# fhausmann/deepgrp

Hardware: AMD Instinct MI355X
Metric: Mbp/sec predicted (whole node) at window=200 stride=50, 5-class (higher is better)
Workload: dtype f16

## Files before the change

deepgrp_amd/csrc/api.hip:

```cpp
#include "dgrp_model.h"

#include <stdarg.h>
#include <string.h>

#include <algorithm>
#include <vector>
#include <mutex>

static thread_local char g_err[512] = "";

void dgrp_set_error(const char *fmt, ...)
{
    va_list ap;
    va_start(ap, fmt);
    vsnprintf(g_err, sizeof(g_err), fmt, ap);
    va_end(ap);
}

DGRP_EXPORT int dgrp_abi_version(void) { return DGRP_ABI_VERSION; }
DGRP_EXPORT const char *dgrp_last_error(void) { return g_err; }

DGRP_EXPORT int dgrp_device_info(char *name, size_t name_cap, int *cu_count, int64_t *hbm_bytes)
{
    int dev = 0;
// ... 553 lines not shown
    if (m->ref_only) {
        *kernel = DGRP_KERNEL_FP32; *lds_bytes = 0; *ospan = 0; *avg_up = 0;
        return DGRP_OK;
    }
    const dgrp_gru_plan plan = dgrp_gru_plan_for(m, mode, step);
    *kernel = (int)plan.kernel; *lds_bytes = (int64_t)plan.lds; *ospan = plan.ospan; *avg_up = plan.avg_up;
    return DGRP_OK;
}

DGRP_EXPORT int dgrp_model_set_precision(dgrp_model *m, int level)
{
    DGRP_REQUIRE(m, "dgrp_model_set_precision: NULL model");
    DGRP_REQUIRE(level == 0 || level == 1, "dgrp_model_set_precision: level must be 0 (fp16 operands) or 1 (split operands)");
    if (m->ref_only) return DGRP_OK;
    DGRP_REQUIRE(level == 0 || m->d_pack_lo || m->d_stream, "dgrp_model_set_precision: this model has no split-operand kernel");
    m->precision = level;
    return DGRP_OK;
}

static int64_t ref_sub_windows(const dgrp_model *m)
{
    const int64_t per = 2 * (int64_t)m->T * m->u * 4 + (int64_t)m->T * (m->C + 1) * 4 + 2 * (int64_t)m->u * 4;
    return std::max<int64_t>(16, std::min<int64_t>(4096, (512ll << 20) / per) / 16 * 16);
}

DGRP_EXPORT int64_t dgrp_forward_workspace_bytes(const dgrp_model *m, int64_t nw)
{
    if (!m || nw < 0) return 0;
    if (m->ref_only) {
        const int64_t sub = std::min<int64_t>(ref_sub_windows(m), std::max<int64_t>(nw, 1));
        return dgrp_align_up(dgrp_forward_reference_workspace_bytes(m, sub), 256) + dgrp_align_up(sub * m->T * (int64_t)m->C * 4, 256);
    }
    if (!m->attention) return 256;
    return dgrp_align_up(nw * m->T * (int64_t)m->UP * 4, 256) + dgrp_align_up(nw * m->T * (int64_t)m->C * 4, 256);
}

static int forward_ref(const dgrp_model *m, const uint8_t *d_idx, int64_t n, int64_t s, dgrp_placement place, int64_t w0, int64_t nw,
                       int merge, float *d_out, void *d_work, int64_t work_bytes, hipStream_t stream)
{
    if (work_bytes < dgrp_forward_workspace_bytes(m, nw) || !d_work) {
        dgrp_set_error("dgrp_forward: this model runs on the fp32 kernels and needs %lld bytes of workspace for %lld windows",
                       (long long)dgrp_forward_workspace_bytes(m, nw), (long long)nw);
        return DGRP_ENOMEM;
    }
    const int64_t sub = std::min<int64_t>(ref_sub_windows(m), nw);
    const int64_t ref_bytes = dgrp_align_up(dgrp_forward_reference_workspace_bytes(m, sub), 256);
    float *probs = (float *)((char *)d_work + ref_bytes);
    for (int64_t a = w0; a < w0 + nw; a += sub) {
        const int64_t k = std::min<int64_t>(sub, w0 + nw - a);
        float *dst = merge ? probs : d_out + (a - w0) * (int64_t)m->T * m->C;
        int rc = dgrp_forward_windows_reference(m, d_idx, n, s, a, k, dst, d_work, ref_bytes, stream);
        if (rc) return rc;
        if (!merge) continue;
        for (int64_t b = a; b < a + k;) {
            const int64_t e = (b < place.nfullB && a + k > place.nfullB) ? place.nfullB : a + k;
            const int64_t row = dgrp_place_row(place, b, s);
            if (row < n) {
                rc = dgrp_get_max(d_out + row * m->C, n - row, probs + (b - a) * (int64_t)m->T * m->C, m->T, m->C, s, e - b, stream);
                if (rc) return rc;
            }
            b = e;
        }
    }
    return DGRP_OK;
}

static int forward_common(const dgrp_model *m, const uint8_t *d_idx, int64_t n, int64_t s, int64_t batch, int64_t w0,
                          int64_t nw, int merge, float *d_out, void *d_work, int64_t work_bytes, hipStream_t stream)
{
    DGRP_REQUIRE(m && s >= 1 && w0 >= 0 && nw >= 0 && n >= 0, "dgrp_forward: bad arguments");
    if (nw == 0) return DGRP_OK;
    DGRP_REQUIRE(d_idx && d_out, "dgrp_forward: NULL pointer");
    DGRP_REQUIRE((w0 + nw - 1) * s + m->T <= n, "dgrp_forward: window %lld (start %lld) runs past n=%lld",
                 (long long)(w0 + nw - 1), (long long)((w0 + nw - 1) * s), (long long)n);
    dgrp_placement place = { 0, 0 };
    if (merge) {
        DGRP_REQUIRE(batch >= 1, "dgrp_forward_merge: batch must be >= 1");
        const int64_t total = dgrp_window_count(n, m->T, s);
        DGRP_REQUIRE(w0 + nw <= total, "dgrp_forward_merge: windows %lld..%lld exceed the record's %lld",
                     (long long)w0, (long long)(w0 + nw), (long long)total);
        place = dgrp_make_placement(total, batch);
    }
    if (m->ref_only) return forward_ref(m, d_idx, n, s, place, w0, nw, merge, d_out, d_work, work_bytes, stream);
    if (!m->attention) return dgrp_gru_launch(m, dgrp_gru_plan_for(m, merge ? 0 : 1, s), d_idx, n, place, w0, nw, d_out, nullptr, stream);
    if (work_bytes < dgrp_forward_workspace_bytes(m, nw) || !d_work) {
        dgrp_set_error("dgrp_forward: attention model needs %lld bytes of workspace for %lld windows",
                       (long long)dgrp_forward_workspace_bytes(m, nw), (long long)nw);
        return DGRP_ENOMEM;
    }
    void *avg = d_work;
    float *pl = (float *)((char *)d_work + dgrp_align_up(nw * m->T * (int64_t)m->UP * 4, 256));
    const dgrp_gru_plan pre = dgrp_gru_plan_for(m, 2, s);
    int rc = dgrp_gru_launch(m, pre, d_idx, n, place, w0, nw, pl, avg, stream);
    if (rc) return rc;
    return dgrp_attention_launch_recs(m, pre, place, w0, nw, merge, n, avg, pl, d_out, nullptr, 0, stream);
}

DGRP_EXPORT int dgrp_forward_windows(const dgrp_model *m, const uint8_t *d_idx, int64_t n, int64_t s, int64_t w0,
                                     int64_t nw, float *d_probs, void *d_work, int64_t work_bytes, void *stream)
{
    return forward_common(m, d_idx, n, s, 1, w0, nw, 0, d_probs, d_work, work_bytes, (hipStream_t)stream);
}

DGRP_EXPORT int dgrp_forward_merge(const dgrp_model *m, const uint8_t *d_idx, int64_t n, int64_t s, int64_t batch,
                                   int64_t w0, int64_t nw, float *d_out, void *d_work, int64_t work_bytes, void *stream)
{
    return forward_common(m, d_idx, n, s, batch, w0, nw, 1, d_out, d_work, work_bytes, (hipStream_t)stream);
}

static int64_t spill_cap_bytes()
{
    static const int64_t cap = [] {
        if (const char *e = getenv("DGRP_SPILL_BYTES")) {
            const long long v = atoll(e);
            if (v >= (1ll << 20)) return (int64_t)v;
        }
        size_t free_b = 0, total_b = 0;
        if (hipMemGetInfo(&free_b, &total_b) != hipSuccess || total_b == 0) return (int64_t)(4ll << 30);
        return std::min<int64_t>(8ll << 30, std::max<int64_t>(1ll << 30, (int64_t)(total_b / 32)));
    }();
    return cap;
}

static int64_t record_window_chunk(const dgrp_model *m)
{
    if (m->ref_only) return ref_sub_windows(m);
// ... 150 lines not shown
        dgrp_set_error("dgrp_predict_record: workspace %lld < %lld bytes", (long long)work_bytes, (long long)l.bytes);
        return DGRP_ENOMEM;
    }
    char *w = (char *)d_work;
    float *out = (float *)(w + l.out);
    int8_t *labels = (int8_t *)(w + l.labels);
    int64_t *d_count = (int64_t *)(w + l.count);
    DGRP_HIP(hipMemsetAsync(out, 0, (size_t)n * m->C * 4, stream));
    int rc = dgrp_forward_merge_record(m, d_idx, n, s, batch, out, w + l.fwd, l.fwd_bytes, stream);
    if (rc) return rc;
    if (use_mss) {
        rc = dgrp_scores(out, n, m->C, (double *)(w + l.scores), (int8_t *)(w + l.cls), stream);
        if (rc) return rc;
        rc = dgrp_mss_labels((const double *)(w + l.scores), (const int8_t *)(w + l.cls), n, m->C, min_mss_len, xdrop_len,
                             labels, nullptr, w + l.post, l.post_bytes, stream);
    } else {
        rc = dgrp_softmax_labels(out, n, m->C, nullptr, labels, w + l.post, l.post_bytes, stream);
    }
    if (rc) return rc;
    rc = dgrp_segments(labels, n, offset, contig, d_records, cap, d_count, w + l.post, l.post_bytes, stream);
    if (rc) return rc;
    DGRP_HIP(hipMemcpyAsync(h_count, d_count, 8, hipMemcpyDeviceToHost, stream));
    DGRP_HIP(hipStreamSynchronize(stream));
    return DGRP_OK;
}

int dgrp_batch_marks(const int64_t *d_start, const int64_t *d_len, int64_t nrec, int64_t total_n, uint8_t *d_marks,
                     double *d_scores, int8_t *d_cls, hipStream_t stream);
int dgrp_batch_segments(const int8_t *d_labels, const uint8_t *d_marks, int64_t total_n, const int64_t *d_start, int64_t nrec,
                        const int64_t *d_startpos, const int32_t *d_contig, dgrp_segment *d_records, int64_t cap,
                        int64_t *d_count, void *d_work, int64_t work_bytes, hipStream_t stream);

struct batch_layout {
    int64_t out, scores, cls, labels, marks, count, recs, wgf, start, len, spos, contig, post, post_bytes, avg, pl, bytes;
};

static batch_layout batch_carve(const dgrp_model *m, int64_t nrec, int64_t total_rows, int64_t total_windows)
{
    batch_layout l;
    int64_t p = 0;
    auto take = [&](int64_t b) { const int64_t q = p; p += dgrp_align_up(b, 256); return q; };
    l.out = take(total_rows * m->C * 4);
    l.scores = take(total_rows * 8);
    l.cls = take(total_rows);
    l.labels = take(total_rows);
    l.marks = take(total_rows);
    l.count = take(8);
    l.recs = take(nrec * 64);
    l.wgf = take((nrec + 1) * 8);
    l.start = take((nrec + 1) * 8);
    l.len = take(nrec * 8);
    l.spos = take(nrec * 8);
    l.contig = take(nrec * 4);
    l.post_bytes = std::max<int64_t>(std::max<int64_t>(dgrp_mss_batch_workspace_bytes(total_rows, nrec), dgrp_segments_workspace_bytes(total_rows)), 4096);
    l.post = take(l.post_bytes);
    l.avg = take(m->attention ? total_windows * m->T * (int64_t)m->UP * 4 : 0);
    l.pl = take(m->attention ? total_windows * m->T * (int64_t)m->C * 4 : 0);
    l.bytes = p;
    return l;
}

static int64_t batch_windows(const dgrp_model *m, int64_t nrec, const int64_t *h_n, int64_t s)
{
    int64_t w = 0;
    for (int64_t r = 0; r < nrec; ++r) w += dgrp_window_count(h_n[r], m->T, s);
    return w;
}

static int64_t batch_rows(int64_t nrec, const int64_t *h_n)
{
    int64_t rows = 0;
    for (int64_t r = 0; r < nrec; ++r) rows += dgrp_align_up(h_n[r], 64);
    return rows;
}

DGRP_EXPORT int64_t dgrp_batch_workspace_bytes(const dgrp_model *m, int64_t nrec, const int64_t *h_n, int64_t s)
{
    if (!m || nrec < 0 || s < 1 || (nrec > 0 && !h_n)) return 0;
    for (int64_t r = 0; r < nrec; ++r)
        if (h_n[r] < 1) return 0;
    return batch_carve(m, nrec, batch_rows(nrec, h_n), batch_windows(m, nrec, h_n, s)).bytes;
}

DGRP_EXPORT int64_t dgrp_batch_rows(int64_t nrec, const int64_t *h_n)
{
    return nrec > 0 && h_n ? batch_rows(nrec, h_n) : 0;
}

static int predict_batch_common(const char *who, const dgrp_model *m, const uint8_t *d_idx, int64_t nrec, const int64_t *h_idx_off,
                                const int64_t *h_n, const int64_t *h_startpos, const int32_t *h_contig, int64_t s,
// ... 9 lines not shown
        DGRP_REQUIRE(h_n[r] >= 1 && h_idx_off[r] >= 0, "%s: record %lld: empty records do not belong in a batch", who, (long long)r);
    const int64_t rows = batch_rows(nrec, h_n);
    DGRP_REQUIRE(rows < (1ll << 31), "%s: %lld rows in one batch (limit 2^31)", who, (long long)rows);
    const int64_t windows = batch_windows(m, nrec, h_n, s);
    DGRP_REQUIRE(windows < (1ll << 31), "%s: too many windows in one batch", who);
    const batch_layout l = batch_carve(m, nrec, rows, windows);
    if (work_bytes < l.bytes) {
        dgrp_set_error("%s: workspace %lld < %lld bytes", who, (long long)work_bytes, (long long)l.bytes);
        return DGRP_ENOMEM;
    }
    char *w = (char *)d_work;
    std::vector<int64_t> recs((size_t)nrec * 8, 0), wgf((size_t)nrec + 1, 0), start((size_t)nrec + 1, 0);
    int64_t wfirst = 0;
    for (int64_t r = 0; r < nrec; ++r) {
        const int64_t nwin = dgrp_window_count(h_n[r], m->T, s);
        const dgrp_placement pl = dgrp_make_placement(nwin, batch);
        int64_t *e = recs.data() + (size_t)r * 8;
        e[0] = h_idx_off[r]; e[1] = h_n[r]; e[2] = start[(size_t)r]; e[3] = nwin; e[4] = pl.nfullB; e[5] = pl.shift; e[6] = wfirst;
        wfirst += nwin;
        wgf[(size_t)r + 1] = wgf[(size_t)r] + (nwin + 15) / 16;
        start[(size_t)r + 1] = start[(size_t)r] + dgrp_align_up(h_n[r], 64);
    }
    DGRP_HIP(hipMemcpyAsync(w + l.recs, recs.data(), recs.size() * 8, hipMemcpyHostToDevice, stream));
    DGRP_HIP(hipMemcpyAsync(w + l.wgf, wgf.data(), wgf.size() * 8, hipMemcpyHostToDevice, stream));
    DGRP_HIP(hipMemcpyAsync(w + l.start, start.data(), start.size() * 8, hipMemcpyHostToDevice, stream));
    DGRP_HIP(hipMemcpyAsync(w + l.len, h_n, (size_t)nrec * 8, hipMemcpyHostToDevice, stream));
    DGRP_HIP(hipMemcpyAsync(w + l.spos, h_startpos, (size_t)nrec * 8, hipMemcpyHostToDevice, stream));
    DGRP_HIP(hipMemcpyAsync(w + l.contig, h_contig, (size_t)nrec * 4, hipMemcpyHostToDevice, stream));
    float *out = d_probs ? d_probs : (float *)(w + l.out);
    DGRP_HIP(hipMemsetAsync(out, 0, (size_t)rows * m->C * 4, stream));
    int rc;
    if (!m->attention) {
        rc = dgrp_gru_launch_batch(m, dgrp_gru_plan_for(m, 0, s), d_idx, w + l.recs, (const int64_t *)(w + l.wgf), nrec, wgf[(size_t)nrec],
                                   out, nullptr, stream);
        if (rc) return rc;
    } else {
        const dgrp_gru_plan pre = dgrp_gru_plan_for(m, 2, s);
        rc = dgrp_gru_launch_batch(m, pre, d_idx, w + l.recs, (const int64_t *)(w + l.wgf), nrec, wgf[(size_t)nrec], (float *)(w + l.pl),
                                   w + l.avg, stream);
        if (rc) return rc;
        rc = dgrp_attention_launch_recs(m, pre, dgrp_placement{ 0, 0 }, 0, windows, 1, rows, w + l.avg, (const float *)(w + l.pl), out,
                                        w + l.recs, nrec, stream);
        if (rc) return rc;
    }
    double *scores = (double *)(w + l.scores);
    int8_t *cls = (int8_t *)(w + l.cls), *labels = (int8_t *)(w + l.labels);
    uint8_t *marks = (uint8_t *)(w + l.marks);
    rc = dgrp_scores(out, rows, m->C, scores, cls, stream);
    if (rc) return rc;
    rc = dgrp_batch_marks((const int64_t *)(w + l.start), (const int64_t *)(w + l.len), nrec, rows, marks, scores, cls, stream);
    if (rc) return rc;
    rc = dgrp_mss_labels_batch(scores, cls, rows, nrec, start.data(), m->C, min_mss_len, xdrop_len, labels, w + l.post, l.post_bytes, stream);
    if (rc) return rc;
    int64_t *d_count = (int64_t *)(w + l.count);
    rc = dgrp_batch_segments(labels, marks, rows, (const int64_t *)(w + l.start), nrec, (const int64_t *)(w + l.spos),
                             (const int32_t *)(w + l.contig), d_records, cap, d_count, w + l.post, l.post_bytes, stream);
    if (rc) return rc;
    DGRP_HIP(hipMemcpyAsync(h_count, d_count, 8, hipMemcpyDeviceToHost, stream));
    DGRP_HIP(hipStreamSynchronize(stream));
    return DGRP_OK;
}

DGRP_EXPORT int dgrp_predict_batch(const dgrp_model *m, const uint8_t *d_idx, int64_t nrec, const int64_t *h_idx_off,
                                   const int64_t *h_n, const int64_t *h_startpos, const int32_t *h_contig, int64_t s,
                                   int64_t batch, int min_mss_len, int xdrop_len, dgrp_segment *d_records, int64_t cap,
                                   int64_t *h_count, void *d_work, int64_t work_bytes, void *stream)
{
    return predict_batch_common("dgrp_predict_batch", m, d_idx, nrec, h_idx_off, h_n, h_startpos, h_contig, s, batch, min_mss_len, xdrop_len,
                                d_records, cap, h_count, d_work, work_bytes, (hipStream_t)stream, nullptr);
}

DGRP_EXPORT int dgrp_predict_batch_probs(const dgrp_model *m, const uint8_t *d_idx, int64_t nrec, const int64_t *h_idx_off,
// ... 10 lines not shown
```

deepgrp_amd/csrc/dgrp_model.h:

```cpp
#pragma once
#include "dgrp_common.h"

struct dgrp_model {
    int T, u, C, attention;
    int cell;
    int onercp;
    int UP;
    int NW;
    int KS;
    int nfrag;
    int precision;
    int is_view;
    int ref_only;
    uint4 *d_pack;
    uint4 *d_pack_lo;
    uint4 *d_pack16;
    float *d_xtab;
    uint4 *d_stream;
    uint4 *d_packw;
    float *d_xtabw;
    int NU16;
    float *d_ffb;
    float *d_scale;
    float *d_wtop;
    float *d_raw;
    int64_t raw_kernel, raw_rec, raw_bias, raw_ffk, raw_ffb, raw_scale;
};

struct dgrp_timer_scope {
    hipStream_t stream;
    int64_t windows;
    hipEvent_t start;
    bool on;
    dgrp_timer_scope(hipStream_t s, int64_t nw);
    ~dgrp_timer_scope();
};

enum class dgrp_kernel { none, wave, split2, stream64, stream, split, lstm, fused };
struct dgrp_gru_plan {
    dgrp_kernel kernel;
    int mode;
    int64_t s;
    size_t lds;
    int ospan, lo_tile_off, xtab_off;
    int avg_up;
};
dgrp_gru_plan dgrp_gru_plan_for(const dgrp_model *m, int mode, int64_t s);
int dgrp_gru_launch(const dgrp_model *m, const dgrp_gru_plan &plan, const uint8_t *d_idx, int64_t n, dgrp_placement place,
                    int64_t w0, int64_t nw, float *d_out, void *d_avg, hipStream_t stream);
struct gru_params;
int dgrp_stream_launch(const gru_params &p, int cell, int NW, int64_t groups, size_t lds, hipStream_t stream);
int dgrp_wave_carve(int NU, gru_params &p, int mode, int64_t s, int64_t budget);
int dgrp_wave_table_bytes(int NU);
int dgrp_wave_launch(const gru_params &p, int NU, int64_t groups, int wave_bytes, bool onercp, hipStream_t stream);
size_t dgrp_stream64_carve(int NW, gru_params &p, int mode, int64_t s, int64_t budget);
int dgrp_stream64_launch(const gru_params &p, int NW, int64_t groups, size_t lds, hipStream_t stream);
int dgrp_gru_launch_batch(const dgrp_model *m, const dgrp_gru_plan &plan, const uint8_t *d_idx, const void *d_recs,
                          const int64_t *d_wg_first, int64_t nrec, int64_t total_groups, float *d_out, void *d_avg, hipStream_t stream);
int dgrp_attention_launch_recs(const dgrp_model *m, const dgrp_gru_plan &pre, dgrp_placement place, int64_t w0, int64_t nw,
                               int merge, int64_t n, const void *d_avg, const float *d_pl, float *d_out,
                               const void *d_recs, int64_t nrec, hipStream_t stream);
```

deepgrp_amd/csrc/gru_kernel.hip:

```cpp
#include "gru_shared.h"
#include <mutex>
template <int NW, int MODE, bool ONERCP>
__global__ void __launch_bounds__(64 * NW, 2) gru_fused_kernel(const gru_params pin)
{
    gru_params p = pin;
    const int64_t bid = wg_record<MODE>(pin, p);
    constexpr int UP = 32 * NW, KS = UP / 16, HS = UP + 8;
    constexpr bool ZSTREAM = NW > 4;
    extern __shared__ __attribute__((aligned(16))) unsigned char smem[];

    const int tid = threadIdx.x;
    const int lane = tid & 63;
    const int wave = __builtin_amdgcn_readfirstlane(tid >> 6);
    const int T = p.T, C = p.C;
    const uint4 *mypack = p.pack + (size_t)wave * p.nfrag * 64 + lane;
    half8 Bz[KS + 1], Br[KS + 1], Bg[KS + 1], Bxh, Bd_hi, Bd_lo;
#pragma unroll
    for (int k = 0; k <= KS; ++k) {
        uint4 a = mypack[(size_t)(k) * 64], b = mypack[(size_t)(KS + 1 + k) * 64], c = mypack[(size_t)(2 * (KS + 1) + k) * 64];
        if (!ZSTREAM || k == KS) Bz[k] = __builtin_bit_cast(half8, a);
        Br[k] = __builtin_bit_cast(half8, b);
        Bg[k] = __builtin_bit_cast(half8, c);
    }
    Bxh = __builtin_bit_cast(half8, mypack[(size_t)(3 * (KS + 1)) * 64]);
// ... 996 lines not shown
        set((const void *)lstm_fused_kernel<NW, 0>);
        set((const void *)lstm_fused_kernel<NW, 1>);
    });
    DGRP_HIP(cfg_err);
    if (p.mode == 0)
        hipLaunchKernelGGL((lstm_fused_kernel<NW, 0>), dim3((unsigned)groups), dim3(64 * NW), lds, stream, p);
    else
        hipLaunchKernelGGL((lstm_fused_kernel<NW, 1>), dim3((unsigned)groups), dim3(64 * NW), lds, stream, p);
    DGRP_LAUNCH_CHECK();
    return DGRP_OK;
}

static size_t gru_tile_carve(const dgrp_model *m, gru_params &p, int mode, int64_t s, bool split, int pad, int64_t budget)
{
    const int lo_tiles = split ? gru_lds_hbuf(m->UP, pad) : 0;
    const int fixed = gru_lds_hbuf(m->UP, pad) + gru_lds_dpart(m->NW) + gru_lds_seq(p.Tp) + gru_lds_meta();
    p.ospan = 0;
    if (mode == 0) {
        const int64_t want = (DGRP_WG_WINDOWS - 1) * s + m->T;
        const int64_t cap = (budget - fixed - lo_tiles) / (m->C * 4);
        p.ospan = (int)(want < cap ? want : cap);
        if (p.ospan < m->T) p.ospan = 0;
    }
    p.lo_tile_off = (int)dgrp_align_up(fixed + (int64_t)p.ospan * m->C * 4, 16);
    return split ? (size_t)p.lo_tile_off + lo_tiles : (size_t)fixed + (size_t)p.ospan * m->C * 4;
}
static int64_t tile_budget(const dgrp_model *m, bool split)
{
    if (m->NW == 1) return 19 * 1024;
    if (m->NW == 2 && split) return 39 * 1024;
    return (m->NW > 4 ? 144 : 72) * 1024;
}
#define DGRP_SPLIT2_PAD 16
#define DGRP_SPLIT2_XTAB_BYTES (5 * (4 * 128 * 4 + 32))

dgrp_gru_plan dgrp_gru_plan_for(const dgrp_model *m, int mode, int64_t s)
{
    gru_params p{};
    p.T = m->T; p.C = m->C; p.Tp = (int)dgrp_align_up(m->T, 16);
    dgrp_gru_plan plan{};
    plan.mode = mode; plan.s = s; plan.avg_up = m->UP;
    auto pick = [&](dgrp_kernel k, size_t lds) {
        plan.kernel = k; plan.lds = lds;
        plan.ospan = p.ospan; plan.lo_tile_off = p.lo_tile_off; plan.xtab_off = p.xtab_off;
        return plan;
    };
    const bool split = (m->cell == 1 && m->NW > 4 && m->d_stream) ||
                       (m->precision == 1 && ((m->cell == 0 && m->NW <= 4 && m->d_pack_lo) || m->d_stream));
    const bool one_tile = getenv("DGRP_SPLIT_ONE_TILE") != nullptr;
    if (split && !one_tile && m->cell == 0 && m->NU16 > 0 && m->d_packw && !(m->NU16 == 2 && mode == 2)) {
        const int64_t budget = (160 * 1024 - dgrp_wave_table_bytes(m->NU16)) / 4 / 16 * 16;
        const int wave_bytes = dgrp_wave_carve(m->NU16, p, mode, s, budget);
        if (wave_bytes <= budget) {
            plan.avg_up = 16 * m->NU16;
            return pick(dgrp_kernel::wave, wave_bytes);
        }
    }
    if (split && !one_tile && m->NW == 4 && m->d_pack16) {
        const int half_bytes = (int)dgrp_align_up((int64_t)gru_tile_carve(m, p, mode, s, true, DGRP_SPLIT2_PAD, 74 * 1024), 256);
        if (2 * half_bytes + DGRP_SPLIT2_XTAB_BYTES <= 160 * 1024) {
            p.xtab_off = 2 * half_bytes;
            return pick(dgrp_kernel::split2, half_bytes);
        }
    }
    const size_t lds = gru_tile_carve(m, p, mode, s, split, 8, tile_budget(m, split));
    if (lds > 160 * 1024) return pick(dgrp_kernel::none, lds);
    if (split && m->d_stream && m->cell == 0 && m->d_xtab) {
// ... 29 lines not shown
        case 3: return launch_split<3>(p, groups, plan.lds, stream);
        default: return launch_split<4>(p, groups, plan.lds, stream);
        }
    case dgrp_kernel::lstm:
        switch (m->NW) {
        case 1: return launch_lstm<1>(p, groups, plan.lds, stream);
        case 2: return launch_lstm<2>(p, groups, plan.lds, stream);
        case 3: return launch_lstm<3>(p, groups, plan.lds, stream);
        case 4: return launch_lstm<4>(p, groups, plan.lds, stream);
        default:
            dgrp_set_error("LSTM units=%d not supported (max 128)", m->u);
            return DGRP_EINVAL;
        }
    case dgrp_kernel::fused:
        switch (m->NW) {
        case 1: return launch_gru<1>(p, groups, plan.lds, onercp, stream);
        case 2: return launch_gru<2>(p, groups, plan.lds, onercp, stream);
        case 3: return launch_gru<3>(p, groups, plan.lds, onercp, stream);
        case 4: return launch_gru<4>(p, groups, plan.lds, onercp, stream);
        case 5: return launch_gru<5>(p, groups, plan.lds, onercp, stream);
        case 6: return launch_gru<6>(p, groups, plan.lds, onercp, stream);
        case 7: return launch_gru<7>(p, groups, plan.lds, onercp, stream);
        case 8: return launch_gru<8>(p, groups, plan.lds, onercp, stream);
        default:
            dgrp_set_error("units=%d not supported by the GRU kernel (max 256)", m->u);
            return DGRP_EINVAL;
        }
    }
    dgrp_set_error("window size %d: the workgroup's staged sequences (%d bytes of LDS) do not fit 160 KiB", m->T, gru_lds_seq(p.Tp));
    return DGRP_EINVAL;
}

int dgrp_gru_launch(const dgrp_model *m, const dgrp_gru_plan &plan, const uint8_t *d_idx, int64_t n, dgrp_placement place,
                    int64_t w0, int64_t nw, float *d_out, void *d_avg, hipStream_t stream)
{
    if (nw <= 0) return DGRP_OK;
    dgrp_timer_scope timed(stream, nw);
    gru_params p{};
    p.idx = d_idx; p.n = n; p.w0 = w0; p.nw = nw; p.place = place; p.out = d_out; p.avg = d_avg;
    const int64_t groups = (nw + DGRP_WG_WINDOWS - 1) / DGRP_WG_WINDOWS;
    DGRP_REQUIRE(groups < (1ll << 31), "too many windows in one launch (%lld)", (long long)nw);
    return gru_dispatch(m, plan, p, groups, stream);
}

int dgrp_gru_launch_batch(const dgrp_model *m, const dgrp_gru_plan &plan, const uint8_t *d_idx, const void *d_recs,
                          const int64_t *d_wg_first, int64_t nrec, int64_t total_groups, float *d_out, void *d_avg, hipStream_t stream)
{
    if (nrec <= 0 || total_groups <= 0) return DGRP_OK;
    dgrp_timer_scope timed(stream, total_groups * DGRP_WG_WINDOWS);
    DGRP_REQUIRE(m->NW <= 8 && (plan.mode == 0 || (plan.mode == 2 && m->cell == 0)), "dgrp_gru_launch_batch: mode 0, or the GRU attention pre-pass");
    gru_params p{};
    p.idx = d_idx; p.out = d_out; p.avg = d_avg;
    p.recs = (const gru_rec *)d_recs; p.wg_first = d_wg_first; p.nrec = nrec;
    DGRP_REQUIRE(total_groups < (1ll << 31), "too many windows in one launch");
    return gru_dispatch(m, plan, p, total_groups, stream);
}

int dgrp_attention_launch_recs(const dgrp_model *m, const dgrp_gru_plan &pre, dgrp_placement place, int64_t w0, int64_t nw,
                               int merge, int64_t n, const void *d_avg, const float *d_pl, float *d_out,
                               const void *d_recs, int64_t nrec, hipStream_t stream)
{
    if (nw <= 0) return DGRP_OK;
    const int64_t s = pre.s;
    att_params p;
    p.avg = d_avg; p.pl = d_pl; p.scale = m->d_scale; p.wtop = m->d_wtop; p.out = d_out;
    p.n = n; p.s = s; p.w0 = w0; p.nw = nw; p.place = place;
    p.T = m->T; p.C = m->C; p.UP = pre.avg_up; p.merge = merge;
    p.recs = (const gru_rec *)d_recs; p.nrec = nrec;
    const int UPs = p.UP;
    const bool f32 = m->precision == 1;
    const int esz = f32 ? 4 : 2;
    DGRP_REQUIRE(nw < (1ll << 31), "too many windows in one launch");
    p.ospan = 0;
    const int64_t want = (ATT_WPB - 1) * s + m->T;
    const unsigned grid = (unsigned)((nw + ATT_WPB - 1) / ATT_WPB);
    if (UPs <= 64) {
        const int stat = 4 * UPs * 2 * 4 + 4 * 64 * (UPs + 16 / esz) * esz;
        if (merge) {
            const int64_t budget = stat <= 40 * 1024 && !f32 ? 78 * 1024 : 156 * 1024;
            const int64_t cap = (budget - stat) / (m->C * 4);
            p.ospan = (int)(want < cap ? want : cap);
            if (p.ospan < m->T) p.ospan = 0;
        }
        const size_t dyn = (size_t)p.ospan * m->C * 4;
        static std::once_flag configured;
// ... 45 lines not shown
```

deepgrp_amd/csrc/gru_shared.h:

```cpp
#pragma once
#include "dgrp_model.h"

typedef _Float16 half8 __attribute__((ext_vector_type(8)));
typedef float f32x16 __attribute__((ext_vector_type(16)));
typedef float f32x4 __attribute__((ext_vector_type(4)));
typedef _Float16 half4 __attribute__((ext_vector_type(4)));

#define DGRP_WG_WINDOWS 16

struct gru_rec {
    int64_t idx_off, n, out_row, nwin;
    dgrp_placement place;
    int64_t win_first;
    int64_t pad_;
};

struct gru_params {
    const uint8_t *idx;
    int64_t n, s, w0, nw;
    dgrp_placement place;
    const uint4 *pack;
    const float *ffb;
    float *out;
    void *avg;
    int avg_f32;
    int T, C, nfrag, mode;
    int Tp;
    int ospan;
    const struct gru_rec *recs;
    const int64_t *wg_first;
    int64_t nrec;
    int64_t avgw;
    const uint4 *pack_lo;
    int lo_tile_off;
    float zfold;
    const uint4 *pack16;
    const float *xtab;
    int xtab_off;
    const uint4 *stream;
    const uint4 *packw;
    const float *xtabw;
    int avg_up;
};

__device__ __forceinline__ float sigmoid_from_scaled(float a) { return __builtin_amdgcn_rcpf(1.0f + __builtin_amdgcn_exp2f(a)); }
__device__ __forceinline__ float tanh_from_scaled(float a) { return 1.0f - 2.0f * __builtin_amdgcn_rcpf(1.0f + __builtin_amdgcn_exp2f(a)); }
typedef float f32x2 __attribute__((ext_vector_type(2)));
__device__ __forceinline__ f32x2 rcp1p_exp2_pair(float a0, float a1)
{
    f32x2 e = { __builtin_amdgcn_exp2f(a0), __builtin_amdgcn_exp2f(a1) };
    e = e + 1.0f;
    return f32x2{ __builtin_amdgcn_rcpf(e.x), __builtin_amdgcn_rcpf(e.y) };
}
__device__ __forceinline__ float fast_tanh(float x) { return tanh_from_scaled(2.8853900817779268f * x); }

template <int N>
__device__ __forceinline__ float row_ror(float x)
{
    return __builtin_bit_cast(float, __builtin_amdgcn_update_dpp(0, __builtin_bit_cast(int, x), 0x120 | N, 0xf, 0xf, false));
}
template <int N>
__device__ __forceinline__ float row_max_ror(float x)
{
    float r;
    asm("s_nop 1\n\tv_max_f32_dpp %0, %1, %1 row_ror:%2 row_mask:0xf bank_mask:0xf" : "=v"(r) : "v"(x), "n"(N));
    return r;
}
template <int CTRL>
__device__ __forceinline__ float quad_perm(float x)
{
    return __builtin_bit_cast(float, __builtin_amdgcn_update_dpp(0, __builtin_bit_cast(int, x), CTRL, 0xf, 0xf, false));
// ... 268 lines not shown
```

deepgrp_amd/csrc/gru_split2.hip:

```cpp
#include "gru_shared.h"
#include <cstddef>
#include <mutex>
#include <type_traits>

typedef unsigned u32x4 __attribute__((ext_vector_type(4)));

namespace {

constexpr int NW = 4, UP = 128, KS = 4, HPAD = 16, HS = UP + HPAD;
constexpr int XT_PITCH = 4 * 128 * 4 + 32;

struct split2_weights {
    u32x4 hi[3][KS][2], lo[3][KS][2];
    u32x4 Bd_hi, Bd_lo;
};

#define LOAD2(a, pa, b, pb)                                                                                             \
    asm volatile("global_load_dwordx4 %0, %2, off\n\tglobal_load_dwordx4 %1, %3, off"                                   \
                 : "=&a"(a), "=&a"(b) : "v"(pa), "v"(pb) : "memory")
#define LOAD_WAIT asm volatile("s_waitcnt vmcnt(0)" ::: "memory")

#define MFMA_R(acc, Wf, b) asm volatile("v_mfma_f32_16x16x32_f16 %0, %1, %2, %0" : "+v"(acc) : "a"(Wf), "v"(b))
#define MFMA_D(acc, a, Wf) asm volatile("v_mfma_f32_16x16x32_f16 %0, %1, %2, %0" : "+v"(acc) : "v"(a), "a"(Wf))
#define MFMA_DZ(acc, a, Wf) asm volatile("v_mfma_f32_16x16x32_f16 %0, %1, %2, 0" : "=&v"(acc) : "v"(a), "a"(Wf))

struct tile_state {
    gru_params p;
    wg_ctx ctx;
    unsigned hcur, hnxt, lcur, lnxt;
    unsigned myseq;
    float h[16];
    f32x4 ar[4], ag[4], az[4], ax[4];
    f32x4 dpl;
    unsigned tabf, tabr;
    half8 f0h[2], f0l[2];
    int p_off;
    int64_t p_row0;
    bool pr_on;
};

__device__ __forceinline__ int64_t split2_uniform(int64_t v)
{
    const unsigned lo = (unsigned)__builtin_amdgcn_readfirstlane((int)(uint64_t)v), hi = (unsigned)__builtin_amdgcn_readfirstlane((int)((uint64_t)v >> 32));
// ... 42 lines not shown
    asm volatile("" : "+v"(z0));
    const uint4 zero = { z0, z0, z0, z0 };
#pragma nounroll
    for (int i = tid; i < 32 * HS * 2 / 16; i += 64 * NW) {
        reinterpret_cast<uint4 *>(base)[i] = zero;
        reinterpret_cast<uint4 *>(base + p.lo_tile_off)[i] = zero;
    }
    c.lo = 0;
    if (MODE == 0) {
        const int64_t a = dgrp_place_row(p.place, c.wg_w, p.s), b = dgrp_place_row(p.place, c.wg_w + c.nvalid - 1, p.s);
        c.lo = split2_uniform(a < b ? a : b);
        const int words = p.ospan * C;
#pragma nounroll
        for (int i = tid; i < words / 4; i += 64 * NW) reinterpret_cast<uint4 *>(c.obuf)[i] = zero;
        if (tid < (words & 3)) c.obuf[(words & ~3) + tid] = 0u;
    }
    if (tid < DGRP_WG_WINDOWS) {
        int64_t r0 = -1;
        int off = -1;
        if (tid < c.nvalid) {
            r0 = MODE == 0 ? dgrp_place_row(p.place, c.wg_w + tid, p.s) : (c.wg_w + tid - p.w0 + p.avgw) * (int64_t)T;
            if (MODE == 0 && r0 >= c.lo && r0 - c.lo + T <= p.ospan) off = (int)(r0 - c.lo);
        }
        c.row0s[tid] = r0;
        c.rowoff[tid] = off;
    }
    return c;
}

struct split2_args {
    gru_params p;
    int half_bytes;
    int npairs;
};

template <int MODE, bool ONERCP>
__global__ void __launch_bounds__(256) __attribute__((amdgpu_waves_per_eu(1, 1))) gru_split2_kernel(const split2_args args)
{
    static_assert(offsetof(split2_args, p) == 0 && sizeof(gru_params) % 4 == 0 && offsetof(split2_args, half_bytes) % 4 == 0 &&
                  offsetof(split2_args, npairs) % 4 == 0, "the pair loop reads the argument as 32-bit words");
    const gru_params &pin = args.p;
    extern __shared__ __attribute__((aligned(16))) unsigned char smem[];
    const int tid = threadIdx.x;
    const int lane = tid & 63;
    const int wave = __builtin_amdgcn_readfirstlane(tid >> 6);
    const int T = pin.T, C = pin.C;

    split2_weights W;
    {
        const uint4 *p16 = pin.pack16 + (size_t)wave * 48 * 64 + lane;
#pragma unroll
        for (int g = 0; g < 3; ++g)
#pragma unroll
            for (int ks = 0; ks < KS; ++ks) {
                LOAD2(W.hi[g][ks][0], p16 + (size_t)(g * 8 + ks * 2) * 64, W.hi[g][ks][1], p16 + (size_t)(g * 8 + ks * 2 + 1) * 64);
                LOAD2(W.lo[g][ks][0], p16 + (size_t)(24 + g * 8 + ks * 2) * 64, W.lo[g][ks][1], p16 + (size_t)(24 + g * 8 + ks * 2 + 1) * 64);
            }
        const uint4 *mypack = pin.pack + (size_t)wave * pin.nfrag * 64 + lane;
        LOAD2(W.Bd_hi, mypack + (size_t)(3 * (2 * KS + 1) + 1) * 64, W.Bd_lo, mypack + (size_t)(3 * (2 * KS + 1) + 2) * 64);
        LOAD_WAIT;
    }
    for (int i = tid; i < 5 * 512; i += 256)
        *reinterpret_cast<float *>(smem + pin.xtab_off + (i / 512) * XT_PITCH + (i % 512) * 4) = pin.xtab[i];

    const int wi = lane & 15, q4 = lane >> 4;
    const int cls = lane & 15;
    const float fbias = cls < C ? pin.ffb[cls] : 0.0f;
    const unsigned frag_lane = (unsigned)(wi * HS + 8 * q4) * 2;
    const unsigned dense_lane = (unsigned)(wi * HS + 32 * wave + 8 * q4) * 2;
    const unsigned pub_lane = (unsigned)(wi * HS + 32 * wave + 4 * q4) * 2;
    const unsigned tab_lane = (unsigned)pin.xtab_off + (unsigned)(32 * wave + 4 * q4) * 4;

    tile_state S0, S1;
    auto setup = [&](tile_state &Z, const gru_params &pk, int tid_k, int half_k, int pair, int x) {
        unsigned char *base = smem + (size_t)x * half_k;
        Z.p = pk;
        const int64_t bid = wg_record_at<MODE>(pk, Z.p, 2 * (int64_t)pair + x);
        unsigned seq_row0, seq_pitch;
        Z.ctx = split2_tile_setup<MODE>(Z.p, base, bid, tid_k, seq_row0, seq_pitch);
// ... 139 lines not shown
#undef RDD
#undef AXL
#undef DS
#undef G
#undef PB
#undef BAR
#undef RD0
#undef XP
#undef CI
#undef FN
    };
    const std::true_type yes;
    const std::false_type no;

    auto first_step = [&](tile_state &Z) {
        tab_rows(Z, smem[Z.myseq], smem[Z.myseq + T - 1]);
#pragma unroll
        for (int g = 0; g < 3; ++g)
#pragma unroll
            for (int sub = 0; sub < 4; ++sub) acc_init(Z, g, sub);
        Z.f0h[0] = lds16(Z.hcur + frag_lane); Z.f0h[1] = lds16(Z.hcur + frag_lane + 16 * HS * 2);
        Z.f0l[0] = lds16(Z.lcur + frag_lane); Z.f0l[1] = lds16(Z.lcur + frag_lane + 16 * HS * 2);
    };
    for (int pair = blockIdx.x;;) {
    const __attribute__((address_space(4))) unsigned *kargs = (const __attribute__((address_space(4))) unsigned *)__builtin_amdgcn_kernarg_segment_ptr();
    asm volatile("" : "+s"(kargs));
    struct { unsigned w[sizeof(gru_params) / 4]; } kraw;
#pragma unroll
    for (unsigned i = 0; i < sizeof(gru_params) / 4; ++i) kraw.w[i] = kargs[offsetof(split2_args, p) / 4 + i];
    const gru_params pk = __builtin_bit_cast(gru_params, kraw);
    const int half_k = (int)kargs[offsetof(split2_args, half_bytes) / 4];
    int tid_k = 64 * wave + lane;
    asm volatile("" : "+v"(tid_k));
    setup(S0, pk, tid_k, half_k, pair, 0);
    setup(S1, pk, tid_k, half_k, pair, 1);
    __syncthreads();
    placement(S0, tid_k);
    placement(S1, tid_k);
    first_step(S0);
    first_step(S1);
    phase(yes, no, no, S0, S1, 0, 0);
#define EDGE_PAD do { asm volatile("s_nop 15\n\ts_nop 7"); __builtin_amdgcn_sched_barrier(0); } while (0)
    EDGE_PAD;
    for (int t = 0; t + 1 < T; ++t) {
        phase(yes, yes, yes, S1, S0, t, t);
        phase(yes, yes, yes, S0, S1, t + 1, t);
        EDGE_PAD;
    }
    phase(yes, yes, yes, S1, S0, T - 1, T - 1);
    phase(no, yes, yes, S0, S1, T, T - 1);

    auto drain = [&](tile_state &Z, bool prev_open, int tid_d) {
        const int lane_d = tid_d & 63;
        const half8 a0 = lds16(Z.hcur + dense_lane), a1 = lds16(Z.hcur + dense_lane + 16 * HS * 2);
        const half8 l0 = lds16(Z.lcur + dense_lane), l1 = lds16(Z.lcur + dense_lane + 16 * HS * 2);
        if (MODE == 2 && (lane_d & 15) < Z.ctx.nvalid) split_avg_store_lane(Z.p, Z.ctx.wg_w, T - 1, UP, wave, lane_d, a0, a1, l0, l1);
        f32x4 d;
        MFMA_DZ(d, a0, W.Bd_hi); MFMA_D(d, a1, W.Bd_hi); MFMA_D(d, a0, W.Bd_lo); MFMA_D(d, a1, W.Bd_lo); MFMA_D(d, l0, W.Bd_hi); MFMA_D(d, l1, W.Bd_hi);
        asm volatile("s_nop 15\n\ts_nop 7" : "+v"(d));
        float *dw = Z.ctx.dpart + ((size_t)((T - 1) & 1) * 4 * NW + wave) * 64 + lane_d;
#pragma unroll
        for (int reg = 0; reg < 4; ++reg) dw[reg * NW * 64] = d[reg];
        __syncthreads();
        if (prev_open && T > 1) finish_register<NW, MODE>(Z.p, Z.ctx, T - 2, wave, fbias, Z.p_off, Z.p_row0, lane_d);
        finish_register<NW, MODE>(Z.p, Z.ctx, T - 1, wave, fbias, Z.p_off, Z.p_row0, lane_d);
        if (MODE == 0 && Z.p.ospan > 0) flush_image<NW>(Z.p, Z.ctx, tid_d);
    };
    int tid_d = 64 * wave + lane;
    asm volatile("" : "+v"(tid_d));
    drain(S0, false, tid_d);
    drain(S1, true, tid_d);
    __syncthreads();
    EDGE_PAD;
    pair += (int)gridDim.x;
    if (pair >= (int)kargs[offsetof(split2_args, npairs) / 4]) break;
    }
}

static int split2_cu_count(int *cus)
{
    static std::mutex mu;
    static int known[64];
    int dev = 0;
    DGRP_HIP(hipGetDevice(&dev));
    std::lock_guard<std::mutex> lock(mu);
    if (dev < 0 || dev >= 64 || known[dev] == 0) {
        int n = 0;
        DGRP_HIP(hipDeviceGetAttribute(&n, hipDeviceAttributeMultiprocessorCount, dev));
        if (n < 1) n = 1;
        if (dev < 0 || dev >= 64) { *cus = n; return DGRP_OK; }
        known[dev] = n;
    }
    *cus = known[dev];
    return DGRP_OK;
}

template <int MODE, bool ONERCP>
int launch_split2(const gru_params &p, int64_t groups, int half_bytes, hipStream_t stream)
{
    static std::once_flag configured;
    static hipError_t cfg_err = hipSuccess;
    std::call_once(configured, [] { cfg_err = hipFuncSetAttribute((const void *)gru_split2_kernel<MODE, ONERCP>, hipFuncAttributeMaxDynamicSharedMemorySize, 160 * 1024); });
    DGRP_HIP(cfg_err);
    const int64_t npairs = (groups + 1) / 2;
    int cus = 0;
    if (const int rc = split2_cu_count(&cus)) return rc;
    const int64_t grid = npairs < cus ? npairs : cus;
    DGRP_REQUIRE(npairs >= 1 && npairs <= 0x7fff0000, "gru_split2_kernel: tile pairs out of range");
    hipLaunchKernelGGL((gru_split2_kernel<MODE, ONERCP>), dim3((unsigned)grid), dim3(256), (size_t)2 * half_bytes + 5 * XT_PITCH, stream, split2_args{ p, half_bytes, (int)npairs });
    DGRP_LAUNCH_CHECK();
    return DGRP_OK;
}

}

int dgrp_split2_launch(const gru_params &p, int64_t groups, int half_bytes, bool onercp, hipStream_t stream)
{
    if (onercp)
        return p.mode == 0 ? launch_split2<0, true>(p, groups, half_bytes, stream)
             : p.mode == 1 ? launch_split2<1, true>(p, groups, half_bytes, stream) : launch_split2<2, true>(p, groups, half_bytes, stream);
    return p.mode == 0 ? launch_split2<0, false>(p, groups, half_bytes, stream)
         : p.mode == 1 ? launch_split2<1, false>(p, groups, half_bytes, stream) : launch_split2<2, false>(p, groups, half_bytes, stream);
}
```

Baseline: 567.6.

## Replace static grid-stride pair walk with atomic work queue in split2 GRU kernel

The persistent split2 GRU kernel now takes its next tile pair from a global atomic counter instead of striding by gridDim.x. Workgroups that finish early can pick up more work, which is meant to even out load across CUs at the tail. The counter lives in a small slot added to the workspace, is zeroed with a memset before each launch, and the next index is shared through LDS. The change adds one atomic per pair plus the memset, and compile-time-gated timestamp instrumentation is added for profiling.

```diff
diff --git a/deepgrp_amd/csrc/api.hip b/deepgrp_amd/csrc/api.hip
--- a/deepgrp_amd/csrc/api.hip
+++ b/deepgrp_amd/csrc/api.hip
@@ -609,7 +609,13 @@
         return dgrp_align_up(dgrp_forward_reference_workspace_bytes(m, sub), 256) + dgrp_align_up(sub * m->T * (int64_t)m->C * 4, 256);
     }
     if (!m->attention) return 256;
-    return dgrp_align_up(nw * m->T * (int64_t)m->UP * 4, 256) + dgrp_align_up(nw * m->T * (int64_t)m->C * 4, 256);
+    return dgrp_align_up(nw * m->T * (int64_t)m->UP * 4, 256) + dgrp_align_up(nw * m->T * (int64_t)m->C * 4, 256) + 256;
+}
+
+static unsigned *forward_queue(const dgrp_model *m, int64_t nw, void *d_work, int64_t work_bytes)
+{
+    if (!d_work || work_bytes < dgrp_forward_workspace_bytes(m, nw)) return nullptr;
+    return (unsigned *)((char *)d_work + (m->attention ? dgrp_forward_workspace_bytes(m, nw) - 256 : 0));
 }
 
 static int forward_ref(const dgrp_model *m, const uint8_t *d_idx, int64_t n, int64_t s, dgrp_placement place, int64_t w0, int64_t nw,
@@ -659,7 +665,9 @@
         place = dgrp_make_placement(total, batch);
     }
     if (m->ref_only) return forward_ref(m, d_idx, n, s, place, w0, nw, merge, d_out, d_work, work_bytes, stream);
-    if (!m->attention) return dgrp_gru_launch(m, dgrp_gru_plan_for(m, merge ? 0 : 1, s), d_idx, n, place, w0, nw, d_out, nullptr, stream);
+    if (!m->attention)
+        return dgrp_gru_launch(m, dgrp_gru_plan_for(m, merge ? 0 : 1, s), d_idx, n, place, w0, nw, d_out, nullptr,
+                               forward_queue(m, nw, d_work, work_bytes), stream);
     if (work_bytes < dgrp_forward_workspace_bytes(m, nw) || !d_work) {
         dgrp_set_error("dgrp_forward: attention model needs %lld bytes of workspace for %lld windows",
                        (long long)dgrp_forward_workspace_bytes(m, nw), (long long)nw);
@@ -668,7 +676,7 @@
     void *avg = d_work;
     float *pl = (float *)((char *)d_work + dgrp_align_up(nw * m->T * (int64_t)m->UP * 4, 256));
     const dgrp_gru_plan pre = dgrp_gru_plan_for(m, 2, s);
-    int rc = dgrp_gru_launch(m, pre, d_idx, n, place, w0, nw, pl, avg, stream);
+    int rc = dgrp_gru_launch(m, pre, d_idx, n, place, w0, nw, pl, avg, forward_queue(m, nw, d_work, work_bytes), stream);
     if (rc) return rc;
     return dgrp_attention_launch_recs(m, pre, place, w0, nw, merge, n, avg, pl, d_out, nullptr, 0, stream);
 }
@@ -885,7 +893,7 @@
                         int64_t *d_count, void *d_work, int64_t work_bytes, hipStream_t stream);
 
 struct batch_layout {
-    int64_t out, scores, cls, labels, marks, count, recs, wgf, start, len, spos, contig, post, post_bytes, avg, pl, bytes;
+    int64_t out, scores, cls, labels, marks, count, recs, wgf, start, len, spos, contig, post, post_bytes, avg, pl, queue, bytes;
 };
 
 static batch_layout batch_carve(const dgrp_model *m, int64_t nrec, int64_t total_rows, int64_t total_windows)
@@ -909,6 +917,7 @@
     l.post = take(l.post_bytes);
     l.avg = take(m->attention ? total_windows * m->T * (int64_t)m->UP * 4 : 0);
     l.pl = take(m->attention ? total_windows * m->T * (int64_t)m->C * 4 : 0);
+    l.queue = take(4);
     l.bytes = p;
     return l;
 }
@@ -984,12 +993,12 @@
     int rc;
     if (!m->attention) {
         rc = dgrp_gru_launch_batch(m, dgrp_gru_plan_for(m, 0, s), d_idx, w + l.recs, (const int64_t *)(w + l.wgf), nrec, wgf[(size_t)nrec],
-                                   out, nullptr, stream);
+                                   out, nullptr, (unsigned *)(w + l.queue), stream);
         if (rc) return rc;
     } else {
         const dgrp_gru_plan pre = dgrp_gru_plan_for(m, 2, s);
         rc = dgrp_gru_launch_batch(m, pre, d_idx, w + l.recs, (const int64_t *)(w + l.wgf), nrec, wgf[(size_t)nrec], (float *)(w + l.pl),
-                                   w + l.avg, stream);
+                                   w + l.avg, (unsigned *)(w + l.queue), stream);
         if (rc) return rc;
         rc = dgrp_attention_launch_recs(m, pre, dgrp_placement{ 0, 0 }, 0, windows, 1, rows, w + l.avg, (const float *)(w + l.pl), out,
                                         w + l.recs, nrec, stream);
diff --git a/deepgrp_amd/csrc/dgrp_model.h b/deepgrp_amd/csrc/dgrp_model.h
--- a/deepgrp_amd/csrc/dgrp_model.h
+++ b/deepgrp_amd/csrc/dgrp_model.h
@@ -47,7 +47,7 @@
 };
 dgrp_gru_plan dgrp_gru_plan_for(const dgrp_model *m, int mode, int64_t s);
 int dgrp_gru_launch(const dgrp_model *m, const dgrp_gru_plan &plan, const uint8_t *d_idx, int64_t n, dgrp_placement place,
-                    int64_t w0, int64_t nw, float *d_out, void *d_avg, hipStream_t stream);
+                    int64_t w0, int64_t nw, float *d_out, void *d_avg, unsigned *d_queue, hipStream_t stream);
 struct gru_params;
 int dgrp_stream_launch(const gru_params &p, int cell, int NW, int64_t groups, size_t lds, hipStream_t stream);
 int dgrp_wave_carve(int NU, gru_params &p, int mode, int64_t s, int64_t budget);
@@ -56,7 +56,8 @@
 size_t dgrp_stream64_carve(int NW, gru_params &p, int mode, int64_t s, int64_t budget);
 int dgrp_stream64_launch(const gru_params &p, int NW, int64_t groups, size_t lds, hipStream_t stream);
 int dgrp_gru_launch_batch(const dgrp_model *m, const dgrp_gru_plan &plan, const uint8_t *d_idx, const void *d_recs,
-                          const int64_t *d_wg_first, int64_t nrec, int64_t total_groups, float *d_out, void *d_avg, hipStream_t stream);
+                          const int64_t *d_wg_first, int64_t nrec, int64_t total_groups, float *d_out, void *d_avg, unsigned *d_queue,
+                          hipStream_t stream);
 int dgrp_attention_launch_recs(const dgrp_model *m, const dgrp_gru_plan &pre, dgrp_placement place, int64_t w0, int64_t nw,
                                int merge, int64_t n, const void *d_avg, const float *d_pl, float *d_out,
                                const void *d_recs, int64_t nrec, hipStream_t stream);
diff --git a/deepgrp_amd/csrc/gru_kernel.hip b/deepgrp_amd/csrc/gru_kernel.hip
--- a/deepgrp_amd/csrc/gru_kernel.hip
+++ b/deepgrp_amd/csrc/gru_kernel.hip
@@ -1052,7 +1052,7 @@
     return (m->NW > 4 ? 144 : 72) * 1024;
 }
 #define DGRP_SPLIT2_PAD 16
-#define DGRP_SPLIT2_XTAB_BYTES (5 * (4 * 128 * 4 + 32))
+#define DGRP_SPLIT2_XTAB_BYTES (5 * (4 * 128 * 4 + 32) + 16)
 
 dgrp_gru_plan dgrp_gru_plan_for(const dgrp_model *m, int mode, int64_t s)
 {
@@ -1148,25 +1148,26 @@
 }
 
 int dgrp_gru_launch(const dgrp_model *m, const dgrp_gru_plan &plan, const uint8_t *d_idx, int64_t n, dgrp_placement place,
-                    int64_t w0, int64_t nw, float *d_out, void *d_avg, hipStream_t stream)
+                    int64_t w0, int64_t nw, float *d_out, void *d_avg, unsigned *d_queue, hipStream_t stream)
 {
     if (nw <= 0) return DGRP_OK;
     dgrp_timer_scope timed(stream, nw);
     gru_params p{};
-    p.idx = d_idx; p.n = n; p.w0 = w0; p.nw = nw; p.place = place; p.out = d_out; p.avg = d_avg;
+    p.idx = d_idx; p.n = n; p.w0 = w0; p.nw = nw; p.place = place; p.out = d_out; p.avg = d_avg; p.queue = d_queue;
     const int64_t groups = (nw + DGRP_WG_WINDOWS - 1) / DGRP_WG_WINDOWS;
     DGRP_REQUIRE(groups < (1ll << 31), "too many windows in one launch (%lld)", (long long)nw);
     return gru_dispatch(m, plan, p, groups, stream);
 }
 
 int dgrp_gru_launch_batch(const dgrp_model *m, const dgrp_gru_plan &plan, const uint8_t *d_idx, const void *d_recs,
-                          const int64_t *d_wg_first, int64_t nrec, int64_t total_groups, float *d_out, void *d_avg, hipStream_t stream)
+                          const int64_t *d_wg_first, int64_t nrec, int64_t total_groups, float *d_out, void *d_avg, unsigned *d_queue,
+                          hipStream_t stream)
 {
     if (nrec <= 0 || total_groups <= 0) return DGRP_OK;
     dgrp_timer_scope timed(stream, total_groups * DGRP_WG_WINDOWS);
     DGRP_REQUIRE(m->NW <= 8 && (plan.mode == 0 || (plan.mode == 2 && m->cell == 0)), "dgrp_gru_launch_batch: mode 0, or the GRU attention pre-pass");
     gru_params p{};
-    p.idx = d_idx; p.out = d_out; p.avg = d_avg;
+    p.idx = d_idx; p.out = d_out; p.avg = d_avg; p.queue = d_queue;
     p.recs = (const gru_rec *)d_recs; p.wg_first = d_wg_first; p.nrec = nrec;
     DGRP_REQUIRE(total_groups < (1ll << 31), "too many windows in one launch");
     return gru_dispatch(m, plan, p, total_groups, stream);
diff --git a/deepgrp_amd/csrc/gru_shared.h b/deepgrp_amd/csrc/gru_shared.h
--- a/deepgrp_amd/csrc/gru_shared.h
+++ b/deepgrp_amd/csrc/gru_shared.h
@@ -37,6 +37,7 @@
     const uint4 *pack16;
     const float *xtab;
     int xtab_off;
+    unsigned *queue;
     const uint4 *stream;
     const uint4 *packw;
     const float *xtabw;
diff --git a/deepgrp_amd/csrc/gru_split2.hip b/deepgrp_amd/csrc/gru_split2.hip
--- a/deepgrp_amd/csrc/gru_split2.hip
+++ b/deepgrp_amd/csrc/gru_split2.hip
@@ -9,6 +9,38 @@
 
 constexpr int NW = 4, UP = 128, KS = 4, HPAD = 16, HS = UP + HPAD;
 constexpr int XT_PITCH = 4 * 128 * 4 + 32;
+constexpr int QUEUE_LDS = 16;
+
+#ifdef DGRP_SPLIT2_STAMPS
+struct split2_stamp_buf { unsigned long long *at; int pairs_cap; int static_walk; };
+split2_stamp_buf g_stamps = { nullptr, 0, 0 };
+#define STAMP_DO(pair_k, slot, clock)                                                                                   \
+    do {                                                                                                                \
+        const unsigned long long t_ = (clock);                                                                          \
+        const __attribute__((address_space(4))) unsigned *ks_ = (const __attribute__((address_space(4))) unsigned *)__builtin_amdgcn_kernarg_segment_ptr(); \
+        asm volatile("" : "+s"(ks_));                                                                                   \
+        unsigned long long *const sb_ = (unsigned long long *)(((uint64_t)ks_[offsetof(split2_args, stamps) / 4 + 1] << 32) | ks_[offsetof(split2_args, stamps) / 4]); \
+        const unsigned cap_ = ks_[offsetof(split2_args, stamp_pairs) / 4];                                              \
+        unsigned *const nrun_ = reinterpret_cast<unsigned *>(smem + ks_[offsetof(gru_params, xtab_off) / 4] + 5 * XT_PITCH + 4); \
+        if (sb_ && wave == 0 && lane == 0) {                                                                            \
+            unsigned long long *const row_ = sb_ + (size_t)blockIdx.x * (3 + 4 * (size_t)cap_);                         \
+            if ((pair_k) < 0) {                                                                                         \
+                if ((slot) == 0) *nrun_ = 0;                                                                            \
+                row_[slot] = t_;                                                                                        \
+                if ((slot) == 1) row_[2] = *nrun_;                                                                      \
+            } else {                                                                                                    \
+                const unsigned n_ = *nrun_;                                                                             \
+                if (n_ < cap_) row_[3 + 4 * (size_t)n_ + (pair_k)] = t_;                                                \
+                if ((pair_k) == 3) *nrun_ = n_ + 1;                                                                     \
+            }                                                                                                           \
+        }                                                                                                               \
+    } while (0)
+#define STAMP(slot, clock) STAMP_DO(-1, slot, clock)
+#define STAMP_PAIR(k) STAMP_DO(k, 0, __builtin_amdgcn_s_memtime())
+#else
+#define STAMP(slot, clock) do { } while (0)
+#define STAMP_PAIR(k) do { } while (0)
+#endif
 
 struct split2_weights {
     u32x4 hi[3][KS][2], lo[3][KS][2];
@@ -117,19 +149,24 @@
     gru_params p;
     int half_bytes;
     int npairs;
+#ifdef DGRP_SPLIT2_STAMPS
+    unsigned long long *stamps;
+    int stamp_pairs;
+#endif
 };
 
 template <int MODE, bool ONERCP>
 __global__ void __launch_bounds__(256) __attribute__((amdgpu_waves_per_eu(1, 1))) gru_split2_kernel(const split2_args args)
 {
     static_assert(offsetof(split2_args, p) == 0 && sizeof(gru_params) % 4 == 0 && offsetof(split2_args, half_bytes) % 4 == 0 &&
-                  offsetof(split2_args, npairs) % 4 == 0, "the pair loop reads the argument as 32-bit words");
+                  offsetof(split2_args, npairs) % 4 == 0 && offsetof(gru_params, queue) % 8 == 0, "the pair loop reads the argument as 32-bit words");
     const gru_params &pin = args.p;
     extern __shared__ __attribute__((aligned(16))) unsigned char smem[];
     const int tid = threadIdx.x;
     const int lane = tid & 63;
     const int wave = __builtin_amdgcn_readfirstlane(tid >> 6);
     const int T = pin.T, C = pin.C;
+    STAMP(0, __builtin_amdgcn_s_memrealtime());
 
     split2_weights W;
     {
@@ -335,6 +372,7 @@
     const int half_k = (int)kargs[offsetof(split2_args, half_bytes) / 4];
     int tid_k = 64 * wave + lane;
     asm volatile("" : "+v"(tid_k));
+    STAMP_PAIR(0);
     setup(S0, pk, tid_k, half_k, pair, 0);
     setup(S1, pk, tid_k, half_k, pair, 1);
     __syncthreads();
@@ -342,6 +380,7 @@
     placement(S1, tid_k);
     first_step(S0);
     first_step(S1);
+    STAMP_PAIR(1);
     phase(yes, no, no, S0, S1, 0, 0);
 #define EDGE_PAD do { asm volatile("s_nop 15\n\ts_nop 7"); __builtin_amdgcn_sched_barrier(0); } while (0)
     EDGE_PAD;
@@ -371,13 +410,27 @@
     };
     int tid_d = 64 * wave + lane;
     asm volatile("" : "+v"(tid_d));
+    STAMP_PAIR(2);
+    const __attribute__((address_space(4))) unsigned *kargs_d = kargs;
+    asm volatile("" : "+s"(kargs_d));
+    typedef __attribute__((address_space(1))) unsigned global_u32;
+    global_u32 *const queue = (global_u32 *)(((uint64_t)kargs_d[offsetof(gru_params, queue) / 4 + 1] << 32) | kargs_d[offsetof(gru_params, queue) / 4]);
+    unsigned *const qword = reinterpret_cast<unsigned *>(smem + kargs_d[offsetof(gru_params, xtab_off) / 4] + 5 * XT_PITCH);
+    const bool ask = queue && tid_d == 0;
+    unsigned nxt;
+    asm volatile("" : "=v"(nxt));
+    if (ask) nxt = __builtin_amdgcn_atomic_inc32(queue, 0xffffffffu, __ATOMIC_RELAXED, "agent");
     drain(S0, false, tid_d);
     drain(S1, true, tid_d);
+    if (ask) *qword = nxt + gridDim.x;
     __syncthreads();
     EDGE_PAD;
-    pair += (int)gridDim.x;
-    if (pair >= (int)kargs[offsetof(split2_args, npairs) / 4]) break;
-    }
+    STAMP_PAIR(3);
+    if (queue) pair = __builtin_amdgcn_readfirstlane((int)*qword);
+    else pair += (int)gridDim.x;
+    if (pair >= (int)kargs_d[offsetof(split2_args, npairs) / 4]) break;
+    }
+    STAMP(1, __builtin_amdgcn_s_memrealtime());
 }
 
 static int split2_cu_count(int *cus)
@@ -410,12 +463,28 @@
     if (const int rc = split2_cu_count(&cus)) return rc;
     const int64_t grid = npairs < cus ? npairs : cus;
     DGRP_REQUIRE(npairs >= 1 && npairs <= 0x7fff0000, "gru_split2_kernel: tile pairs out of range");
-    hipLaunchKernelGGL((gru_split2_kernel<MODE, ONERCP>), dim3((unsigned)grid), dim3(256), (size_t)2 * half_bytes + 5 * XT_PITCH, stream, split2_args{ p, half_bytes, (int)npairs });
+    split2_args a{ p, half_bytes, (int)npairs };
+    if (npairs <= grid) a.p.queue = nullptr;
+#ifdef DGRP_SPLIT2_STAMPS
+    if (g_stamps.static_walk) a.p.queue = nullptr;
+    a.stamps = g_stamps.at;
+    a.stamp_pairs = g_stamps.pairs_cap;
+#endif
+    if (a.p.queue) DGRP_HIP(hipMemsetAsync(a.p.queue, 0, sizeof(unsigned), stream));
+    hipLaunchKernelGGL((gru_split2_kernel<MODE, ONERCP>), dim3((unsigned)grid), dim3(256), (size_t)2 * half_bytes + 5 * XT_PITCH + QUEUE_LDS, stream, a);
     DGRP_LAUNCH_CHECK();
     return DGRP_OK;
 }
 
 }
+
+#ifdef DGRP_SPLIT2_STAMPS
+extern "C" __attribute__((visibility("default"))) int dgrp_split2_stamps(void *d_buf, int pairs_cap, int static_walk)
+{
+    g_stamps = { (unsigned long long *)d_buf, pairs_cap, static_walk };
+    return DGRP_OK;
+}
+#endif
 
 int dgrp_split2_launch(const gru_params &p, int64_t groups, int half_bytes, bool onercp, hipStream_t stream)
 {
```

Measured after the change: 577.1 (median of 6 runs). 1.02x the previous value.
